# mako443/Text2Pos-CVPR2022

Measured on AMD Instinct MI355X. Metric: cells+queries encoded/sec and top-k retrieval QPS, 256-pt cells, 12k-cell DB, higher is better.
Workload: dtype f16x3 (fp32 operands split hi+lo into fp16, 3 f16 MFMAs, fp32 accumulate; fp32-class error) for the encoders / f64 MFMA for the ranking

## Files before the change

### include/t2p.h

```cpp
#ifndef T2P_H
#define T2P_H
#include <stddef.h>
#include <stdint.h>

#ifdef __cplusplus
extern "C" {
#endif

#define T2P_ABI_VERSION 29
#define T2P_DEFAULT_CHUNK_OBJECTS 65000
#define T2P_MAX_CHUNK_OBJECTS 65535
#define T2P_TUNING_MASK 0x1
#define T2P_E_ARG (-1)
#define T2P_E_WORKSPACE (-2)
#define T2P_E_UNSUPPORTED (-3)

typedef void* t2p_stream_t;

int t2p_abi_version(void);
const char* t2p_last_error(void);

typedef struct t2p_cell_weights {
    const float* sa_w1[3];
    const float* sa_b1[3];
    const float* sa_w2[3];
    const float* sa_b2[3];
    const float* ga_w1;
    const float* ga_b1;
    const float* ga_w2;
    const float* ga_b2;
    const float* lin1_w;
    const float* lin1_b;
    const float* lin2_w;
    const float* lin2_b;
    const float* pn_w;
    const float* pn_b;
    const float* col_w1;
    const float* col_b1;
    const float* col_w2;
    const float* col_b2;
    const float* pos_w1;
    const float* pos_b1;
    const float* pos_w2;
    const float* pos_b2;
    const float* merge_w;
    const float* merge_b;
    const float* g_wp;
    const float* g_bp;
    const float* g_wq;
    const float* g_w2;
    const float* g_b2;
    const float* lin_w1;
    const float* lin_b1;
    const float* lin_w2;
    const float* lin_b2;
    const void* sa_w2_x3[3];
    const void* ga_w2_x3;
    const float* sa_b2_x3[3];
    float sa_w2_scale[3];
    const void* lin1_x3;
    const void* lin2_x3;
    const void* merge_x3;
    const void* pn_x3;
    const void* g_wp_x3;
    const void* g_wq_x3;
// ... 189 lines not shown
```

### text2pos-cvpr2022_amd/csrc/api.hip

```cpp
#include <stdarg.h>
#include <stdlib.h>
#include <string.h>

#include <mutex>
#include <set>
#include <utility>

#include "../../include/t2p.h"
#include "t2p_common.h"

namespace t2p {

static thread_local char g_err[512] = "";

void set_error(const char* fmt, ...) {
    va_list ap;
    va_start(ap, fmt);
    vsnprintf(g_err, sizeof(g_err), fmt, ap);
    va_end(ap);
}

int num_cus() {
    static int cached = 0;
    if (cached == 0) {
// ... 294 lines not shown
            p.W_x3 = cfg.precision == 1 ? W.sa_w1_x3[l] : nullptr;
            p.ldw = H;
            p.bias = W.sa_b1[l];
            p.out = ws.A[l];
            p.ldo = H;
            p.relu = 0;
            p.M = n * g.nd[l];
            p.amax_out = gslot(l == 1 ? G_A2 : G_A3);
            T2P_TRY(launch_ws(WS_DENSE_STORE, Geo::LD[l - 1] - (cfg.precision == 1 ? 16 : 0), H, p, st));
        }
        SaParams p{};
        p.A = ws.A[l];
        p.Bc = ws.B[l];
        p.wp = lds_btab[l] ? W.sa_w1[l] + (size_t)cf * Geo::H[l] : nullptr;
        p.W = W.sa_w2[l];
        p.W_x3 = cfg.precision == 1 ? W.sa_w2_x3[l] : nullptr;
        p.bias = cfg.precision == 1 ? W.sa_b2_x3[l] : W.sa_b2[l];
        p.out_scale = cfg.precision == 1 ? 1.0f / W.sa_w2_scale[l] : 1.0f;
        p.out = ws.F[l];
        p.ldo = Geo::LD[l];
        p.rows = ws.gt.rows[l];
        p.n_rows = ws.gt.n_rows[l];
        p.first = ws.first;
        p.fps_idx = ws.gt.fps_idx[l];
        p.pos_src = pos_src;
        p.ld_pos = ld_pos;
        p.pos_col0 = pos_col0;
        if (l == 0 && sa1_points) {
            p.feat_src = rgb;
            p.w1 = W.sa_w1[0];
            p.b1 = W.sa_b1[0];
        }
        p.n_dense = g.nd[l];
        p.n_cent = g.nc[l];
        p.n_obj = n;
        p.prefix_ws = ws.prefix[l];
        p.bounds_ws = ws.bounds[l];
        p.balanced = 1;
        p.amax_out = gslot(G_F1 + l);
        if (l == 2) p.out_rows = g.gp;
        T2P_TRY(launch_ws_sa(H, C, p, st));
    }
    {
        WsParams p{};
        p.A = ws.F[2];
        p.lda = Geo::LD[2];
        p.W = W.ga_w1;
        p.W_x3 = cfg.precision == 1 ? W.ga_w1_x3 : nullptr;
        p.ldw = 512;
        p.bias = W.ga_b1;
        p.out = ws.gh;
        _Float16* gh_hi = (_Float16*)ws.gh;
        _Float16* gh_lo = gh_hi + (size_t)gh_rows(n, g) * 512;
        if (cfg.precision == 1) {
            p.out_hi = gh_hi;
            p.out_lo = gh_lo;
            p.amax_out = gslot(G_GA_H);
        }
        p.ldo = 512;
        p.relu = 1;
        p.M = n * g.gp;
        T2P_TRY(launch_ws(WS_DENSE_STORE, Geo::LD[2] - (cfg.precision == 1 ? 16 : 0), 512, p, st));
        WsParams q{};
        q.A = ws.gh;
        if (cfg.precision == 1) {
            q.A_hi = gh_hi;
            q.A_lo = gh_lo;
        }
        q.lda = 512;
        q.W = W.ga_w2;
        q.W_x3 = cfg.precision == 1 ? W.ga_w2_x3 : nullptr;
        q.ldw = 1024;
        q.bias = W.ga_b2;
        q.out = ws.f0;
        q.ldo = 1024;
        q.relu = 1;
        q.M = n * g.gp;
        q.group_rows = g.gp;
        T2P_TRY(launch_ws(WS_DENSE_GROUPMAX, 512, 1024, q, st));
    }
    if (cfg.precision == 1 && W.lin1_x3 && W.lin2_x3) {
        T2P_TRY(launch_gemm_x3(ws.f0, 1024, W.lin1_x3, W.lin1_scale, W.lin1_b, ws.f1, 512, 0, n, 1024, 512, 1, st, nullptr, 0, gslot(G_PN_F0)));
        T2P_TRY(launch_gemm_x3(ws.f1, 512, W.lin2_x3, W.lin2_scale, W.lin2_b, ws.f2, 256, 0, n, 512, 256, 1, st, nullptr, 0, gslot(G_PN_F1)));
    } else {
        T2P_TRY(launch_gemm(ws.f0, 1024, W.lin1_w, W.lin1_b, ws.f1, 512, 0, n, 1024, 512, 1, st));
        T2P_TRY(launch_gemm(ws.f1, 512, W.lin2_w, W.lin2_b, ws.f2, 256, 0, n, 512, 256, 1, st));
    }
    }
    if (trunk_only) {
        T2P_TRY(copy_trace(tr->features0, ws.f0, (size_t)n * 1024, st));
        T2P_TRY(copy_trace(tr->features1, ws.f1, (size_t)n * 512, st));
        T2P_TRY(copy_trace(tr->features2, ws.f2, (size_t)n * 256, st));
        T2P_TRY(launch_guard_check(guard, cfg.overflow_flag, gbounds, st));
        return 0;
    }
    const int nfeat = (cfg.use_class ? 1 : 0) + (cfg.use_color ? 1 : 0) + (cfg.use_position ? 1 : 0);
    const int ldcat = nfeat * D;
    int slot = 0;
    if (cfg.use_class && cfg.class_embed) {
        T2P_TRY(launch_gather_rownorm(W.class_embedding, cfg.class_idx + o_lo, n, D, ws.cat, ldcat, slot * D, st));
        slot++;
    } else if (cfg.use_class) {
        const float* fin = cfg.pointnet_features == 0 ? ws.f0 : (cfg.pointnet_features == 1 ? ws.f1 : ws.f2);
        const int kin = cfg.pointnet_features == 0 ? 1024 : (cfg.pointnet_features == 1 ? 512 : 256);
        if (cfg.precision == 1 && W.pn_x3)
            T2P_TRY(launch_gemm_x3(fin, kin, W.pn_x3, W.pn_scale, W.pn_b, ws.P, D, 0, n, kin, D, 1, st, nullptr, 0,
                                          gslot(G_PN_F0 + cfg.pointnet_features)));
        else
            T2P_TRY(launch_gemm(fin, kin, W.pn_w, W.pn_b, ws.P, D, 0, n, kin, D, 1, st));
        T2P_TRY(launch_rownorm(ws.P, D, n, D, ws.cat, ldcat, slot * D, st));
        slot++;
    }
    if (cfg.use_color && cfg.color_embed) {
        T2P_TRY(launch_gather_rownorm(W.color_embedding, cfg.color_idx + o_lo, n, D, ws.cat, ldcat, slot * D, st));
        slot++;
    } else if (cfg.use_color) {
        T2P_TRY(launch_mlp3_norm(mean_rgb, n, W.col_w1, W.col_b1, W.col_w2, W.col_b2, D, ws.cat, ldcat, slot * D, st));
        slot++;
    }
    if (cfg.use_position) {
// ... 643 lines not shown
```

### text2pos-cvpr2022_amd/csrc/ga2.hip

```cpp
#include "t2p_common.h"

namespace t2p {
namespace {

typedef _Float16 half8 __attribute__((ext_vector_type(8)));

constexpr int K = 512, NW = 128, NT = 512;
constexpr int KH = K / 2;
constexpr int S16_FULL = K / 16;
constexpr int LDHH = K + 8;
constexpr int PLANE = 32 * LDHH;
constexpr int TILE_HALVES = 2 * PLANE;
constexpr int XCH_FLOATS = 4 * 16 * 64;
constexpr size_t kLds = (size_t)2 * TILE_HALVES * 2 + (size_t)XCH_FLOATS * 4;
constexpr int CHUNKS = (2 * 32 * (K / 8)) / NT;

template <int GP>
__global__ __launch_bounds__(NT, 2) void k_ga2(WsParams p, int n_slices) {
    extern __shared__ __attribute__((aligned(16))) float lds[];
    _Float16* tile = (_Float16*)lds;
    float* xch = (float*)(tile + 2 * TILE_HALVES);

    const int tid = threadIdx.x, lane = tid & 63, wave = tid >> 6;
    const int wn = wave & 3, kh = wave >> 2;

    const int lin = blockIdx.x, nblk = gridDim.x;
    int slice, stream, n_streams;
    if ((nblk % (8 * n_slices)) == 0) {
        const int xcd = lin & 7, j = lin >> 3, per_xcd = nblk >> 3;
        slice = j % n_slices;
        stream = xcd * (per_xcd / n_slices) + j / n_slices;
        n_streams = nblk / n_slices;
    } else {
        slice = lin % n_slices;
        stream = lin / n_slices;
        n_streams = nblk / n_slices;
    }
    const int ncol0 = slice * NW + wn * 32;

    constexpr int S32 = KH / 32;
    const int q16 = lane >> 4, i16 = lane & 15;
    half8 w_hi[2][S32], w_lo[2][S32];
    {
        const uint4* wp = (const uint4*)p.W_x3;
        const int plane_u4 = (p.ldw / 32) * S16_FULL * 64;
#pragma unroll
        for (int cb = 0; cb < 2; cb++)
#pragma unroll
            for (int s = 0; s < S32; s++) {
                const int idx = (((ncol0 / 32) * S16_FULL + (8 * q16 + s)) * 2 + kh) * 32 + 16 * cb + i16;
                w_hi[cb][s] = __builtin_bit_cast(half8, wp[idx]);
                w_lo[cb][s] = __builtin_bit_cast(half8, wp[plane_u4 + idx]);
            }
    }
    float bias2[2];
#pragma unroll
    for (int cb = 0; cb < 2; cb++) bias2[cb] = p.bias ? p.bias[ncol0 + 16 * cb + i16] : 0.f;

    typedef __attribute__((address_space(3))) void lds_void;
    typedef const __attribute__((address_space(1))) void gl_void;
    auto dma_piece = [&](int64_t g, int buf, int it) {
        const int q = it * (NT / 64) + wave;
        const int pl = q >> 5, row = q & 31;
        const _Float16* base = (const _Float16*)(pl ? p.A_lo : p.A_hi);
        const _Float16* src = base + (g * 32 + row) * (int64_t)p.lda + lane * 8;
        _Float16* dst = tile + buf * TILE_HALVES + pl * PLANE + row * LDHH;
        __builtin_amdgcn_global_load_lds((gl_void*)src, (lds_void*)dst, 16, 0, 0);
    };
    auto dma_tile = [&](int64_t g, int buf) {
#pragma unroll
        for (int it = 0; it < CHUNKS; it++) dma_piece(g, buf, it);
    };
    int64_t g = stream;
    if (g < p.n_groups) dma_tile(g, 0);
    __syncthreads();
    for (int i = 0; g < p.n_groups; g += n_streams, i++) {
        const int64_t gn = g + n_streams;
        const bool more = gn < p.n_groups;

        typedef float f32x4v __attribute__((ext_vector_type(4)));
        const f32x4v kZero4 = {0.f, 0.f, 0.f, 0.f};
        f32x4v acc[4], accx[4];
        const _Float16* hrow = tile + (i & 1) * TILE_HALVES + i16 * LDHH + kh * KH + q16 * 64;
        half8 a_hi[2], a_lo[2];
#pragma unroll
        for (int rb = 0; rb < 2; rb++) {
            a_hi[rb] = *(const half8*)(hrow + rb * 16 * LDHH);
            a_lo[rb] = *(const half8*)(hrow + PLANE + rb * 16 * LDHH);
        }
#pragma unroll
        for (int sl = 0; sl < 4 * S32; sl++) {
            const int s = sl >> 2, b = sl & 3, rb = b >> 1, cb = b & 1;
            __builtin_amdgcn_sched_barrier(0);
            if (s + 1 < S32 && b == 2) {
                a_hi[0] = *(const half8*)(hrow + (s + 1) * 8);
                a_lo[0] = *(const half8*)(hrow + PLANE + (s + 1) * 8);
            }
            if (s > 0 && b == 0) {
                a_hi[1] = *(const half8*)(hrow + 16 * LDHH + s * 8);
                a_lo[1] = *(const half8*)(hrow + PLANE + 16 * LDHH + s * 8);
            }
            acc[b] = __builtin_amdgcn_mfma_f32_16x16x32_f16(a_hi[rb], w_hi[cb][s], s == 0 ? kZero4 : acc[b], 0, 0, 0);
            accx[b] = __builtin_amdgcn_mfma_f32_16x16x32_f16(a_hi[rb], w_lo[cb][s], s == 0 ? kZero4 : accx[b], 0, 0, 0);
            accx[b] = __builtin_amdgcn_mfma_f32_16x16x32_f16(a_lo[rb], w_hi[cb][s], accx[b], 0, 0, 0);
            __builtin_amdgcn_sched_barrier(0);
            if (more && (sl & 1) == 0 && (sl >> 1) < CHUNKS) dma_piece(gn, (i + 1) & 1, sl >> 1);
        }
        __builtin_amdgcn_sched_barrier(0);
#pragma unroll
        for (int b = 0; b < 4; b++)
#pragma unroll
            for (int v = 0; v < 4; v++) acc[b][v] = fmaf(accx[b][v], 1.f / 2048.f, acc[b][v]);
        float* x = xch + wn * (16 * 64) + lane;
        const bool sender = ((i & 1) != 0) == (kh == 0);
        if (sender) {
#pragma unroll
            for (int b = 0; b < 4; b++)
#pragma unroll
                for (int v = 0; v < 4; v++) x[(4 * b + v) * 64] = acc[b][v];
        }
        __syncthreads();
        if (!sender && GP == 32) {
#pragma unroll
            for (int cb = 0; cb < 2; cb++) {
                float m = 0.f;
#pragma unroll
                for (int rb = 0; rb < 2; rb++)
#pragma unroll
                    for (int v = 0; v < 4; v++) m = fmaxf(m, (acc[2 * rb + cb][v] + x[(4 * (2 * rb + cb) + v) * 64]) + bias2[cb]);
                m = fmaxf(m, __shfl_xor(m, 16, 64));
                m = fmaxf(m, __shfl_xor(m, 32, 64));
                if (q16 == 0) p.out[g * (int64_t)p.ldo + ncol0 + 16 * cb + i16] = m;
            }
        } else if (!sender) {
            constexpr int VG = GP < 4 ? GP : 4;
            const int64_t n_obj = p.M / GP;
#pragma unroll
            for (int cb = 0; cb < 2; cb++)
#pragma unroll
                for (int rb = 0; rb < 2; rb++)
#pragma unroll
                    for (int v0 = 0; v0 < 4; v0 += VG) {
                        float m = 0.f;
#pragma unroll
                        for (int v = v0; v < v0 + VG; v++)
                            m = fmaxf(m, (acc[2 * rb + cb][v] + x[(4 * (2 * rb + cb) + v) * 64]) + bias2[cb]);
                        if constexpr (GP >= 8) m = fmaxf(m, __shfl_xor(m, 16, 64));
                        if constexpr (GP >= 16) m = fmaxf(m, __shfl_xor(m, 32, 64));
                        const int row = 16 * rb + 4 * q16 + v0;
                        const int64_t obj = g * (32 / GP) + row / GP;
                        if (row % GP == 0 && obj < n_obj) p.out[obj * (int64_t)p.ldo + ncol0 + 16 * cb + i16] = m;
                    }
        }
    }
}

template <int GP>
int launch_ga2_gp(const WsParams& p_in, hipStream_t st) {
    T2P_TRY(reserve_lds((const void*)k_ga2<GP>, kLds, "ga2"));
    WsParams p = p_in;
    p.n_groups = (p.M + 31) / 32;
    if (p.n_groups <= 0) return 0;
    const int n_slices = 1024 / NW;
    int64_t streams = matrix_wgs() / n_slices;
    if (streams < 1) streams = 1;
    if (streams > p.n_groups) streams = p.n_groups;
    if (streams >= 8) streams -= streams % 8;
    ProfScope ps_("ws_groupmax_k512_n1024", st);
    T2P_REPEAT(ps_) hipLaunchKernelGGL(k_ga2<GP>, dim3((unsigned)(streams * n_slices)), dim3(NT), kLds, st, p, n_slices);
    T2P_CHECK_LAUNCH("ga2");
    return 0;
}

}

int launch_ga2(const WsParams& p, hipStream_t st) {
    switch (p.group_rows > 0 ? p.group_rows : 32) {
        case 32: return launch_ga2_gp<32>(p, st);
        case 16: return launch_ga2_gp<16>(p, st);
        case 8: return launch_ga2_gp<8>(p, st);
        case 4: return launch_ga2_gp<4>(p, st);
        case 2: return launch_ga2_gp<2>(p, st);
        case 1: return launch_ga2_gp<1>(p, st);
    }
    set_error("ga2: group_rows=%d (1, 2, 4, 8, 16 or 32)", p.group_rows);
    return T2P_E_UNSUPPORTED;
}

}
```

### text2pos-cvpr2022_amd/csrc/t2p_common.h

```cpp
#pragma once
#include <hip/hip_runtime.h>
#include <stdint.h>
#include <stdio.h>

namespace t2p {

void set_error(const char* fmt, ...);

#define T2P_E_ARG (-1)
#define T2P_E_WORKSPACE (-2)
#define T2P_E_UNSUPPORTED (-3)

#define T2P_CHECK_ARG(cond, ...)                  \
    do {                                          \
        if (!(cond)) {                            \
            ::t2p::set_error(__VA_ARGS__);        \
            return T2P_E_ARG;                     \
        }                                         \
    } while (0)

#define T2P_CHECK_LAUNCH(name)                                                   \
    do {                                                                         \
        hipError_t e__ = hipGetLastError();                                      \
        if (e__ != hipSuccess) {                                                 \
// ... 123 lines not shown
    float* A1;
    const float* w1;
    const float* b1;
    const float* rgb;
    int H1;
    uint32_t* guard;
};
int launch_sample_group(const float* xyz, int64_t n_obj, int n_pts, const float radius[3], GroupTables gt,
                        hipStream_t st);
int launch_dedup_rows(const float* xyz, const float* rgb, int64_t n_obj, int n_pts, uint16_t* rows, uint16_t* n_rows,
                      int n_cent, hipStream_t st);

int launch_rownorm(const float* in, int ld_in, int64_t n_rows, int dim, float* out, int ld_out, int col0,
                   hipStream_t st);
int launch_gather_rownorm(const float* table, const int32_t* idx, int64_t n_rows, int dim, float* out, int ld_out,
                          int col0, hipStream_t st);
int launch_segmax(const float* in, int dim, const int32_t* seg_ptr, int n_seg, float* out, int mean,
                  hipStream_t st);
int launch_knn(const float* x, int dim, const int32_t* seg_ptr, int n_seg, int max_seg_rows, int k,
               int32_t* out_idx, hipStream_t st);
int launch_mlp3_norm(const float* in3, int64_t n_rows, const float* w1, const float* b1, const float* w2,
                     const float* b2, int D, float* out, int ld_out, int col0, hipStream_t st);
int launch_pack_objects(const float* raw_xyz, const float* raw_rgb, const int32_t* obj_ptr, const int32_t* sample_idx,
                        const float* rot, int64_t n_obj, int n_pts, float* xyz, float* rgb, float* center, float* mean_rgb,
                        hipStream_t st);
int launch_pack_scene(const float* raw_xyz, const float* raw_rgb, const int32_t* obj_ptr, const int32_t* obj_id, const uint64_t* key,
                      const float* scene_center, const float* scene_color, int64_t n_out, int n_pts, float* xyz, float* rgb,
                      float* center, float* mean_rgb, int32_t* idx_out, hipStream_t st);
int launch_pairwise_ranking(const float* scores, int batch, float margin, float* row_loss, float* d_scores, float* row_cnt,
                            hipStream_t st);
int launch_hardest_ranking(const float* scores, int batch, float margin, float* best, int32_t* where, float* d_scores,
                           hipStream_t st);
int launch_cell_index(const int32_t* cell_ptr, int n_cells, int32_t o_lo, int32_t* seg_ptr_local, int32_t* first,
                      hipStream_t st, uint32_t* guard_to_clear = nullptr);

int launch_gemm(const float* A, int lda, const float* W, const float* bias, float* C, int ldc, int c0, int64_t M,
                int K, int N, int relu, hipStream_t st, const float* resid = nullptr, int ldr = 0);
int launch_gemm_skinny(const float* A, int lda, const float* W, float* C, int ldc, int64_t M, int K, int N, hipStream_t st);
int launch_gemm_x3(const float* A, int lda, const void* Wx, float scale, const float* bias, float* C, int ldc, int c0,
                   int64_t M, int K, int N, int relu, hipStream_t st, const float* resid = nullptr, int ldr = 0,
                   uint32_t* amax_in = nullptr );

size_t gemm_tn_workspace_bytes(int64_t M, int K1, int N);
int launch_edge_counts(const uint16_t* rows, const uint16_t* n_rows, const int32_t* first_obj, int64_t n_obj, int n_dense, int n_cent,
                       int self_loops, int32_t* counts, hipStream_t st);
int launch_edge_expand(const uint16_t* rows, const uint16_t* n_rows, const int32_t* first_obj, const int32_t* cent_ptr, int64_t n_obj,
                       int n_dense, int n_cent, int self_loops, int32_t* src, int32_t* dst, hipStream_t st);
size_t linear_wgrad_workspace_bytes(int64_t M, int K1, int N);
int launch_linear_wgrad_f32(const float* dY, int lda, const float* X, int ldb, float* dW, int ldc, float* colsum, int64_t M, int K1, int N,
                            void* ws, size_t ws_bytes, hipStream_t st);
int launch_gemm_tn(const float* A, int lda, const float* B, int ldb, float* C, int ldc, int64_t M, int K1, int N, void* ws,
                   size_t ws_bytes, hipStream_t st);

enum WsMode { WS_DENSE_STORE = 0, WS_DENSE_GROUPMAX = 1, WS_EDGE_KNN = 3 };
struct WsParams {
    const float* A;
    int lda;
    int k_live;
    const float* Bc;
    const float* W;
    int ldw;
    const void* W_x3;
    const void* A_hi;
    const void* A_lo;
    void* out_hi;
    void* out_lo;
    const float* bias;
    float* out;
    int ldo;
    int relu;
    int64_t n_groups;
    int64_t M;
    uint32_t* amax_out;
    const int32_t* knn_idx;
    int knn_k;
    int64_t n_dst;
    int mean;
    int knn_group;
    int group_rows;
};
int launch_ws(int mode, int K, int N, const WsParams& p, hipStream_t st);

struct SaParams {
    const float* A;
    const float* Bc;
    const float* wp;
    const float* W;
    const void* W_x3;
    const float* bias;
    float out_scale;
    float* out;
    int ldo;
    const uint16_t* rows;
    const uint16_t* n_rows;
    const int32_t* first;
    const uint8_t* fps_idx;
    const float* pos_src;
    int ld_pos, pos_col0;
    const float* feat_src;
    const float* w1;
    const float* b1;
    int n_dense, n_cent;
    int64_t n_obj;
    int32_t* prefix_ws;
    int32_t* bounds_ws;
    int balanced;
    uint32_t* amax_out;
    int out_rows;
};
int launch_ws_sa(int H, int C, const SaParams& p, hipStream_t st);
int launch_sa_x3(int H, int C, const SaParams& p, hipStream_t st);
int sa_x3_launch_shape(int H, int C, int64_t n_obj, int* tile_rows, int* n_wg);
bool sa_rows_selected(int H, int C, const SaParams& p);
int launch_sa_rows(int H, int C, const SaParams& p, hipStream_t st);
int sa_rows_launch_shape(int64_t n_obj, int* tile_rows, int* n_wg);
bool sa_points_selected(int H, int C, const SaParams& p);
int launch_sa_points(int H, int C, const SaParams& p, hipStream_t st);
int sa_points_launch_shape(int64_t n_obj, int* tile_rows, int* n_wg);
bool sa3_selected(int H, int C, const SaParams& p);
// ... 48 lines not shown
```

### text2pos-cvpr2022_amd/csrc/ws_gemm.hip

```cpp
#ifndef T2P_GABL
#define T2P_GABL 0
#endif
#ifndef T2P_GA2_V1
#define T2P_GA2_V1 0
#endif
#include <type_traits>

#include "t2p_common.h"

namespace t2p {
namespace {

typedef _Float16 half8 __attribute__((ext_vector_type(8)));
typedef __fp16 fp16x2 __attribute__((ext_vector_type(2)));

constexpr int kMaxRows = 32 * 33;
constexpr int kAccFloats = 8192;

template <int K, int NW, int WN, int RT, int MODE, int X3, int W8 = 0>
struct WsCfg {
    static constexpr int NWAVES = (WN > 4 || W8) ? 8 : 4;
    static constexpr int NTH = 64 * NWAVES;
    static constexpr int WM = NWAVES / WN;
    static constexpr int NTW = NW / (32 * WN);
// ... 51 lines not shown
    half8 w_hi[X3 ? C::NTW : 1][X3 ? C::S16 : 1], w_lo[X3 ? C::NTW : 1][X3 ? C::S16 : 1];
    if constexpr (X3) {
        const uint4* wp = (const uint4*)p.W_x3;
        const int plane_u4 = (p.ldw / 32) * C::S16 * 64;
#pragma unroll
        for (int nt = 0; nt < C::NTW; nt++)
#pragma unroll
            for (int s = 0; s < C::S16; s++) {
                const int idx = (((ncol0 / 32 + nt) * C::S16 + s) * 2 + h) * 32 + l31;
                const uint4 a = wp[idx], b = wp[plane_u4 + idx];
                w_hi[nt][s] = __builtin_bit_cast(half8, a);
                w_lo[nt][s] = __builtin_bit_cast(half8, b);
            }
    } else {
#pragma unroll
        for (int nt = 0; nt < C::NTW; nt++)
#pragma unroll
            for (int s = 0; s < C::KS; s++)
                w[nt][s] = p.W[(int64_t)(h * C::KS + s) * p.ldw + ncol0 + nt * 32 + l31];
    }
    float bias[C::NTW];
#pragma unroll
    for (int nt = 0; nt < C::NTW; nt++) bias[nt] = p.bias ? p.bias[ncol0 + nt * 32 + l31] : 0.f;

    const int k_live = p.k_live > 0 ? p.k_live : K;
    f32x4 sa[C::ITERS];
    f32x4 sb[C::EDGE ? C::ITERS : 1];

    const int knn_group = (C::EDGE && p.knn_group > 0) ? p.knn_group : 32;
    auto stage_load = [&](int64_t g, int r0, int n_rows) {
#pragma unroll
        for (int it = 0; it < C::ITERS; it++) {
            const int q = it * C::NTH + tid;
            const int lr = q / C::F4_PER_ROW, c4 = q % C::F4_PER_ROW;
            const int r = r0 + lr;
            sa[it] = f32x4{0.f, 0.f, 0.f, 0.f};
            if constexpr (C::EDGE) sb[it] = f32x4{0.f, 0.f, 0.f, 0.f};
            if (((C::TOTAL_F4 % C::NTH) == 0 || q < C::TOTAL_F4) && (r < n_rows || SPLIT_IO == 1)) {
                if constexpr (C::EDGE) {
                    const int src = rows_src[r];
                    const int dl = rows_dst[r];
                    if (dl != 0xFF) {
                        sa[it] = *(const f32x4*)(p.A + (int64_t)src * p.lda + c4 * 4);
                        sb[it] = *(const f32x4*)(p.Bc + (g * knn_group + dl) * K + c4 * 4);
                    }
                } else if constexpr (SPLIT_IO == 1) {
                    constexpr int CH_PER_PLANE = C::TR * (K / 8);
                    const int pl = q / CH_PER_PLANE, idx = q % CH_PER_PLANE;
                    const int prow = idx / (K / 8), c8 = idx % (K / 8);
                    const _Float16* base = (const _Float16*)(pl ? p.A_lo : p.A_hi);
                    sa[it] = f32x4{0.f, 0.f, 0.f, 0.f};
                    if (prow < n_rows) sa[it] = *(const f32x4*)(base + (g * C::TR + prow) * (int64_t)p.lda + c8 * 8);
                } else {
                    if (SPLIT_IO == 2 || c4 * 4 < k_live)
                        sa[it] = *(const f32x4*)(p.A + (g * C::TR + r) * (int64_t)p.lda + c4 * 4);
                }
            }
        }
    };
    float gmax_edge = 0.f;
    auto stage_write = [&](int buf) {
#pragma unroll
        for (int it = 0; it < C::ITERS; it++) {
            const int q = it * C::NTH + tid;
            if ((C::TOTAL_F4 % C::NTH) != 0 && q >= C::TOTAL_F4) break;
            const int lr = q / C::F4_PER_ROW, c4 = q % C::F4_PER_ROW;
            f32x4 v = sa[it];
            if constexpr (C::EDGE) {
                const f32x4 t = sa[it] + sb[it];
#pragma unroll
                for (int e = 0; e < 4; e++) v[e] = fmaxf(t[e], 0.f);
            }
            if constexpr (X3 && SPLIT_IO == 1) {
                constexpr int CH_PER_PLANE = C::TR * (K / 8);
                const int pl = q / CH_PER_PLANE, idx = q % CH_PER_PLANE;
                const int prow = idx / (K / 8), c8 = idx % (K / 8);
                *(f32x4*)(hidh + buf * 2 * C::PLANE + pl * C::PLANE + prow * C::LDHH + c8 * 8) = sa[it];
            } else if constexpr (X3) {
                _Float16* dsth = hidh + buf * 2 * C::PLANE;
                if constexpr (C::EDGE)
                    gmax_edge = fmaxf(fmaxf(gmax_edge, fmaxf(v[0], v[1])), fmaxf(v[2], v[3]));
                const fp16x2 h01 = cvt_pk_f16(v[0], v[1]), h23 = cvt_pk_f16(v[2], v[3]);
                const fp16x2 l01 = cvt_pk_f16((v[0] - (float)h01[0]) * 2048.f, (v[1] - (float)h01[1]) * 2048.f);
                const fp16x2 l23 = cvt_pk_f16((v[2] - (float)h23[0]) * 2048.f, (v[3] - (float)h23[1]) * 2048.f);
                uint2 ph, pl;
                ph.x = __builtin_bit_cast(uint32_t, h01); ph.y = __builtin_bit_cast(uint32_t, h23);
                pl.x = __builtin_bit_cast(uint32_t, l01); pl.y = __builtin_bit_cast(uint32_t, l23);
                *(uint2*)(dsth + lr * C::LDHH + c4 * 4) = ph;
                *(uint2*)(dsth + C::PLANE + lr * C::LDHH + c4 * 4) = pl;
            } else {
                *(f32x4*)(hid + buf * C::TILE_FLOATS + lr * C::LDH + c4 * 4) = v;
            }
        }
    };
    auto mfma_block = [&](int buf, f32x16 (&acc)[RT][C::NTW]) {
#pragma unroll
        for (int rt = 0; rt < RT; rt++)
#pragma unroll
            for (int nt = 0; nt < C::NTW; nt++)
#pragma unroll
                for (int e = 0; e < 16; e++) acc[rt][nt][e] = bias[nt];
        if constexpr (X3) {
            f32x16 accx[RT][C::NTW];
#pragma unroll
            for (int rt = 0; rt < RT; rt++)
#pragma unroll
                for (int nt = 0; nt < C::NTW; nt++)
// ... 50 lines not shown
#pragma unroll
                for (int rt = 0; rt < RT; rt++) a[rt] = *(const f32x4*)(hrow + rt * 32 * C::LDH + s4 * 4);
#pragma unroll
                for (int j = 0; j < 4; j++)
#pragma unroll
                    for (int rt = 0; rt < RT; rt++)
#pragma unroll
                        for (int nt = 0; nt < C::NTW; nt++)
                            acc[rt][nt] = __builtin_amdgcn_mfma_f32_32x32x2f32(a[rt][j], w[nt][s4 * 4 + j], acc[rt][nt],
                                                                                0, 0, 0);
            }
        }
    };

    if constexpr (!C::EDGE) {
        int64_t g = stream;
        auto rows_of = [&](int64_t gg) -> int {
            const int64_t left = p.M - gg * C::TR;
            return (int)(left < C::TR ? left : C::TR);
        };
        if (g < p.n_groups) {
            stage_load(g, 0, rows_of(g));
            stage_write(0);
        }
        __syncthreads();
        float gmax_all = 0.f;
        (void)gmax_all;
        for (int i = 0; g < p.n_groups; g += n_streams, i++) {
            const int64_t gn = g + n_streams;
            const int n_rows = rows_of(g);
            if (gn < p.n_groups) stage_load(gn, 0, rows_of(gn));
            f32x16 acc[RT][C::NTW];
            mfma_block(i & 1, acc);
            float gmax_out = 0.f;
            (void)gmax_out;
            auto epilogue = [&](auto full_tag) {
            constexpr bool FULL = decltype(full_tag)::value;
#pragma unroll
            for (int rt = 0; rt < RT; rt++) {
                const int trow0 = (wm * RT + rt) * 32;
#pragma unroll
                for (int nt = 0; nt < C::NTW; nt++) {
                    const int lcol = wn * C::NTW * 32 + nt * 32 + l31;
                    if constexpr (MODE == WS_DENSE_STORE) {
                        const int64_t o0 = (g * C::TR + trow0 + 4 * h) * (int64_t)p.ldo + slice * NW + lcol;
#pragma unroll
                        for (int e = 0; e < 16; e++) {
                            const int rr = (e & 3) + 8 * (e >> 2);
                            const int r = trow0 + 4 * h + rr;
                            float v = acc[rt][nt][e];
                            if (p.relu) v = fmaxf(v, 0.f);
                            if constexpr (X3) gmax_out = fmaxf(gmax_out, fabsf(v));
                            if constexpr (SPLIT_IO == 2) {
                                const fp16x2 hv = cvt_pk_f16(v, 0.f);
                                const fp16x2 lv = cvt_pk_f16((v - (float)hv[0]) * 2048.f, 0.f);
#if T2P_GABL & 1
                                if (FULL || r < n_rows) {
                                    ((__fp16*)p.out_hi + (o0 & 0xFFFFF))[rr * p.ldo] = hv[0];
                                    ((__fp16*)p.out_lo + (o0 & 0xFFFFF))[rr * p.ldo] = lv[0];
                                }
#else
                                if (FULL || r < n_rows) {
                                    ((__fp16*)p.out_hi + o0)[rr * p.ldo] = hv[0];
                                    ((__fp16*)p.out_lo + o0)[rr * p.ldo] = lv[0];
                                }
#endif
                            } else {
                                if (FULL || r < n_rows) (p.out + o0)[rr * p.ldo] = v;
                            }
                        }
                    } else if constexpr (GP == 32) {
                        float m = 0.f;
#pragma unroll
                        for (int e = 0; e < 16; e++) m = fmaxf(m, acc[rt][nt][e]);
                        m = fmaxf(m, __shfl_xor(m, 32, 64));
                        if (h == 0 && (FULL || trow0 < n_rows))
                            p.out[(g * (C::TR / 32) + wm * RT + rt) * (int64_t)p.ldo + slice * NW + lcol] = m;
                    } else {
                        constexpr int NG = 32 / GP;
                        float mg[NG];
#pragma unroll
                        for (int k = 0; k < NG; k++) mg[k] = 0.f;
#pragma unroll
                        for (int e = 0; e < 16; e++) {
                            const int k = (8 * (e >> 2) + (GP >= 8 ? 0 : (e & 3))) / GP;
                            mg[k] = fmaxf(mg[k], acc[rt][nt][e]);
                        }
                        const int64_t obj0 = (g * C::TR + trow0) / GP, n_obj = p.M / GP;
#pragma unroll
                        for (int k = 0; k < NG; k++) {
                            if constexpr (GP >= 8) {
                                const float m = fmaxf(mg[k], __shfl_xor(mg[k], 32, 64));
                                if (h == 0 && obj0 + k < n_obj) p.out[(obj0 + k) * (int64_t)p.ldo + slice * NW + lcol] = m;
                            } else if ((k * GP) % 8 < 4) {
                                const int64_t obj = obj0 + k + (4 / GP) * h;
                                if (obj < n_obj) p.out[obj * (int64_t)p.ldo + slice * NW + lcol] = mg[k];
                            }
                        }
                    }
                }
            }
            };
            if (n_rows == C::TR) epilogue(std::true_type{});
            else epilogue(std::false_type{});
            if constexpr (X3 && MODE == WS_DENSE_STORE) gmax_all = fmaxf(gmax_all, gmax_out);
            if (gn < p.n_groups) stage_write((i + 1) & 1);
            __syncthreads();
        }
        if constexpr (X3 && MODE == WS_DENSE_STORE) guard_publish_exact(p.amax_out, gmax_all);
    } else {
        for (int64_t g = stream; g < p.n_groups; g += n_streams) {
            const int64_t d0 = g * knn_group;
            const int nd = (int)((p.n_dst - d0) < knn_group ? (p.n_dst - d0) : knn_group);
            int my = 0;
            if (tid < nd)
                for (int e = 0; e < p.knn_k; e++) my += p.knn_idx[(d0 + tid) * p.knn_k + e] >= 0 ? 1 : 0;
            if (tid <= 32) scan[tid] = 0;
            __syncthreads();
            if (tid < 32) scan[tid + 1] = my;
// ... 79 lines not shown
                        for (int e = 0; e < 16; e++)
                            if (is_end[e]) atomicMax(&acc_lds[dd[e] * NW + lcol], __float_as_int(v[e]));
                    }
                }
                if (more) stage_write((bt + 1) & 1);
                __syncthreads();
            }
            for (int i = tid; i < nd * NW; i += C::NTH) {
                const int c = i / NW, col = i % NW;
                p.out[(d0 + c) * (int64_t)p.ldo + slice * NW + col] = __int_as_float(acc_lds[i]);
            }
            __syncthreads();
        }
        if constexpr (X3) guard_publish_exact(p.amax_out, gmax_edge);
    }
}

template <int K, int NW, int WN, int RT, int MODE, int X3, int SPLIT_IO, int W8 = 0, int GP = 32>
int launch_cfg(const WsParams& p_in, int n_slices, hipStream_t st) {
    using C = WsCfg<K, NW, WN, RT, MODE, X3, W8>;
    auto kern = k_ws<K, NW, WN, RT, MODE, X3, SPLIT_IO, W8, GP>;
    T2P_TRY(reserve_lds((const void*)kern, C::lds_bytes(), "ws_gemm"));
    WsParams p = p_in;
    if (MODE != WS_EDGE_KNN) p.n_groups = (p.M + C::TR - 1) / C::TR;
    if (p.n_groups <= 0) return 0;
    const int cus = num_cus();
    int64_t streams = cus / n_slices;
    if (streams < 1) streams = 1;
    if (streams > p.n_groups) streams = p.n_groups;
    if (streams >= 8) streams -= streams % 8;
    const unsigned grid = (unsigned)(streams * n_slices);
    static const char* kMode[] = {"dense", "groupmax", "edge_sa", "edge_knn"};
    static char name[64];
    if (name[0] == 0) snprintf(name, sizeof(name), "ws_%s_k%d_n%d", kMode[MODE], K, NW * n_slices);
    ProfScope ps_(name, st);
    T2P_REPEAT(ps_) hipLaunchKernelGGL(kern, dim3(grid), dim3(C::NTH), C::lds_bytes(), st, p, n_slices);
    T2P_CHECK_LAUNCH("ws_gemm");
    return 0;
}

}

int launch_ga2(const WsParams& p, hipStream_t st);

int launch_ws(int mode, int K, int N, const WsParams& p, hipStream_t st) {
    T2P_CHECK_ARG((((uintptr_t)p.A | (uintptr_t)p.A_hi | (uintptr_t)p.A_lo) & 15) == 0 && (p.lda % 4) == 0,
                  "ws_gemm: A must be 16-byte aligned, lda %% 4 == 0");
    const int x3 = p.W_x3 != nullptr ? 1 : 0;
    if (x3) T2P_CHECK_ARG(((uintptr_t)p.W_x3 & 15) == 0, "ws_gemm: packed f16x3 weights must be 16-byte aligned");
    const int gp = p.group_rows > 0 ? p.group_rows : 32;
    if (mode == WS_DENSE_GROUPMAX)
        T2P_CHECK_ARG(gp <= 32 && (gp & (gp - 1)) == 0 && p.M % gp == 0, "ws_gemm: groupmax needs group_rows in {1, 2, 4, 8, 16, 32} "
                      "and M %% group_rows == 0 (group_rows=%d M=%lld)", p.group_rows, (long long)p.M);
    const int split_io = p.A_hi != nullptr ? 1 : (p.out_hi != nullptr ? 2 : 0);
    T2P_CHECK_ARG(split_io == 0 || x3 == 1, "ws_gemm: split fp16 activations need the f16x3 path");
    T2P_CHECK_ARG(p.k_live == 0 || (split_io == 0 && mode == WS_DENSE_STORE && p.k_live % 4 == 0),
                  "ws_gemm: k_live is honoured by the fp32-in / fp32-out dense mode only (multiple of 4)");
    if (split_io == 1) T2P_CHECK_ARG(p.A_lo != nullptr && p.lda % 8 == 0, "ws_gemm: split input needs both planes, lda %% 8 == 0");
    if (split_io == 2) T2P_CHECK_ARG(p.out_lo != nullptr, "ws_gemm: split output needs both planes");
#define WS_CASE(MODE_, K_, N_, NW_, WN_, RT_, X3_, SIO_)                                      \
    if (mode == MODE_ && K == K_ && N == N_ && x3 == X3_ && split_io == SIO_)                  \
        return launch_cfg<K_, NW_, WN_, RT_, MODE_, X3_, SIO_>(p, N_ / NW_, st);
    WS_CASE(WS_EDGE_KNN, 256, 256, 256, 8, 1, 0, 0)
    WS_CASE(WS_EDGE_KNN, 256, 256, 256, 8, 1, 1, 0)
    WS_CASE(WS_EDGE_KNN, 128, 128, 128, 4, 1, 0, 0)
    WS_CASE(WS_EDGE_KNN, 128, 128, 128, 4, 1, 1, 0)
    WS_CASE(WS_EDGE_KNN, 384, 384, 128, 4, 1, 0, 0)
    WS_CASE(WS_EDGE_KNN, 384, 384, 128, 4, 1, 1, 0)
    WS_CASE(WS_DENSE_STORE, 96, 128, 128, 4, 2, 0, 0)
    WS_CASE(WS_DENSE_STORE, 160, 256, 256, 4, 1, 0, 0)
    WS_CASE(WS_DENSE_STORE, 288, 512, 128, 4, 1, 0, 0)
    if (mode == WS_DENSE_STORE && K == 80 && N == 128 && x3 == 1 && split_io == 0)
        return launch_cfg<80, 128, 4, 1, WS_DENSE_STORE, 1, 0, 1>(p, 1, st);
    WS_CASE(WS_DENSE_STORE, 144, 256, 256, 8, 1, 1, 0)
    WS_CASE(WS_DENSE_STORE, 272, 512, 256, 8, 1, 1, 2)
    if (mode == WS_DENSE_GROUPMAX && K == 512 && N == 1024 && x3 == 0 && split_io == 0) {
        switch (gp) {
            case 32: return launch_cfg<512, 128, 4, 1, WS_DENSE_GROUPMAX, 0, 0>(p, 8, st);
            case 16: return launch_cfg<512, 128, 4, 1, WS_DENSE_GROUPMAX, 0, 0, 0, 16>(p, 8, st);
            case 8: return launch_cfg<512, 128, 4, 1, WS_DENSE_GROUPMAX, 0, 0, 0, 8>(p, 8, st);
            case 4: return launch_cfg<512, 128, 4, 1, WS_DENSE_GROUPMAX, 0, 0, 0, 4>(p, 8, st);
            case 2: return launch_cfg<512, 128, 4, 1, WS_DENSE_GROUPMAX, 0, 0, 0, 2>(p, 8, st);
            case 1: return launch_cfg<512, 128, 4, 1, WS_DENSE_GROUPMAX, 0, 0, 0, 1>(p, 8, st);
        }
    }
#if !T2P_GA2_V1
    if (mode == WS_DENSE_GROUPMAX && K == 512 && N == 1024 && x3 == 1 && split_io == 1) return launch_ga2(p, st);
#endif
    T2P_CHECK_ARG(mode != WS_DENSE_GROUPMAX || gp == 32, "ws_gemm: group_rows=%d is built for the fp32 and the ga2.hip paths", gp);
    WS_CASE(WS_DENSE_GROUPMAX, 512, 1024, 128, 4, 1, 1, 1)
#undef WS_CASE
    set_error("ws_gemm: no instantiation for mode=%d K=%d N=%d x3=%d split_io=%d", mode, K, N, x3, split_io);
    return T2P_E_UNSUPPORTED;
}

}
```

Measured before the change: 148,900.

## Store GA hidden fp16 planes in swizzled line-blocked tiles for ga2 loads

Changes the layout of the split hi/lo fp16 hidden activations between the two GA layers. Instead of row-major planes, they are stored as 32-row by 512-column tiles made of 32x32 blocks with an XOR swizzle. The producer GEMM writes them with buffer stores, and the ga2 group-max kernel DMA-loads each tile as contiguous memory into LDS, where it reads the operand pieces without bank conflicts and without row padding. The old row-major path stays available behind tuning bit 4. The risk is that the producer's scattered 2-byte stores become less coalesced.

```diff
diff --git a/include/t2p.h b/include/t2p.h
--- a/include/t2p.h
+++ b/include/t2p.h
@@ -10,7 +10,7 @@
 #define T2P_ABI_VERSION 29
 #define T2P_DEFAULT_CHUNK_OBJECTS 65000
 #define T2P_MAX_CHUNK_OBJECTS 65535
-#define T2P_TUNING_MASK 0x1
+#define T2P_TUNING_MASK 0x5
 #define T2P_E_ARG (-1)
 #define T2P_E_WORKSPACE (-2)
 #define T2P_E_UNSUPPORTED (-3)
diff --git a/text2pos-cvpr2022_amd/csrc/api.hip b/text2pos-cvpr2022_amd/csrc/api.hip
--- a/text2pos-cvpr2022_amd/csrc/api.hip
+++ b/text2pos-cvpr2022_amd/csrc/api.hip
@@ -370,9 +370,11 @@
         p.out = ws.gh;
         _Float16* gh_hi = (_Float16*)ws.gh;
         _Float16* gh_lo = gh_hi + (size_t)gh_rows(n, g) * 512;
+        const int gh_rowmajor = (cfg.tuning & 4) ? 1 : 0;
         if (cfg.precision == 1) {
             p.out_hi = gh_hi;
             p.out_lo = gh_lo;
+            p.plane_rowmajor = gh_rowmajor;
             p.amax_out = gslot(G_GA_H);
         }
         p.ldo = 512;
@@ -384,6 +386,7 @@
         if (cfg.precision == 1) {
             q.A_hi = gh_hi;
             q.A_lo = gh_lo;
+            q.plane_rowmajor = gh_rowmajor;
         }
         q.lda = 512;
         q.W = W.ga_w2;
diff --git a/text2pos-cvpr2022_amd/csrc/ga2.hip b/text2pos-cvpr2022_amd/csrc/ga2.hip
--- a/text2pos-cvpr2022_amd/csrc/ga2.hip
+++ b/text2pos-cvpr2022_amd/csrc/ga2.hip
@@ -9,14 +9,19 @@
 constexpr int KH = K / 2;
 constexpr int S16_FULL = K / 16;
 constexpr int LDHH = K + 8;
-constexpr int PLANE = 32 * LDHH;
-constexpr int TILE_HALVES = 2 * PLANE;
 constexpr int XCH_FLOATS = 4 * 16 * 64;
-constexpr size_t kLds = (size_t)2 * TILE_HALVES * 2 + (size_t)XCH_FLOATS * 4;
 constexpr int CHUNKS = (2 * 32 * (K / 8)) / NT;
-
-template <int GP>
+static_assert(K == kGaPlaneCols, "the line-blocked planes are K columns wide");
+template <bool LINES>
+struct Tile {
+    static constexpr int PLANE = LINES ? kGaTileHalves : 32 * LDHH;
+    static constexpr int TILE_HALVES = 2 * PLANE;
+    static constexpr size_t kLds = (size_t)2 * TILE_HALVES * 2 + (size_t)XCH_FLOATS * 4;
+};
+
+template <int GP, bool LINES>
 __global__ __launch_bounds__(NT, 2) void k_ga2(WsParams p, int n_slices) {
+    constexpr int PLANE = Tile<LINES>::PLANE, TILE_HALVES = Tile<LINES>::TILE_HALVES;
     extern __shared__ __attribute__((aligned(16))) float lds[];
     _Float16* tile = (_Float16*)lds;
     float* xch = (float*)(tile + 2 * TILE_HALVES);
@@ -63,8 +68,9 @@
         const int q = it * (NT / 64) + wave;
         const int pl = q >> 5, row = q & 31;
         const _Float16* base = (const _Float16*)(pl ? p.A_lo : p.A_hi);
-        const _Float16* src = base + (g * 32 + row) * (int64_t)p.lda + lane * 8;
-        _Float16* dst = tile + buf * TILE_HALVES + pl * PLANE + row * LDHH;
+        const _Float16* src = LINES ? base + g * kGaTileHalves + row * (kGaBlockHalves / 2) + lane * 8
+                                    : base + (g * 32 + row) * (int64_t)p.lda + lane * 8;
+        _Float16* dst = tile + buf * TILE_HALVES + pl * PLANE + row * (LINES ? kGaBlockHalves / 2 : LDHH);
         __builtin_amdgcn_global_load_lds((gl_void*)src, (lds_void*)dst, 16, 0, 0);
     };
     auto dma_tile = [&](int64_t g, int buf) {
@@ -82,23 +88,32 @@
         const f32x4v kZero4 = {0.f, 0.f, 0.f, 0.f};
         f32x4v acc[4], accx[4];
         const _Float16* hrow = tile + (i & 1) * TILE_HALVES + i16 * LDHH + kh * KH + q16 * 64;
+        const _Float16* hpc[4];
+#pragma unroll
+        for (int pc = 0; pc < 4; pc++)
+            hpc[pc] = tile + (i & 1) * TILE_HALVES + ((kh * KH + q16 * 64) / 32) * kGaBlockHalves + ga_block_off(i16, 8 * pc);
+        static_assert(ga_block_off(16, 0) == kGaBlockHalves / 2, "rows 16-31 of a block follow rows 0-15");
+        auto opnd = [&](int s, int rb, int pl) -> half8 {
+            if constexpr (LINES) return *(const half8*)(hpc[s & 3] + pl * PLANE + rb * (kGaBlockHalves / 2) + (s >> 2) * kGaBlockHalves);
+            else return *(const half8*)(hrow + pl * PLANE + rb * 16 * LDHH + s * 8);
+        };
         half8 a_hi[2], a_lo[2];
 #pragma unroll
         for (int rb = 0; rb < 2; rb++) {
-            a_hi[rb] = *(const half8*)(hrow + rb * 16 * LDHH);
-            a_lo[rb] = *(const half8*)(hrow + PLANE + rb * 16 * LDHH);
+            a_hi[rb] = opnd(0, rb, 0);
+            a_lo[rb] = opnd(0, rb, 1);
         }
 #pragma unroll
         for (int sl = 0; sl < 4 * S32; sl++) {
             const int s = sl >> 2, b = sl & 3, rb = b >> 1, cb = b & 1;
             __builtin_amdgcn_sched_barrier(0);
             if (s + 1 < S32 && b == 2) {
-                a_hi[0] = *(const half8*)(hrow + (s + 1) * 8);
-                a_lo[0] = *(const half8*)(hrow + PLANE + (s + 1) * 8);
+                a_hi[0] = opnd(s + 1, 0, 0);
+                a_lo[0] = opnd(s + 1, 0, 1);
             }
             if (s > 0 && b == 0) {
-                a_hi[1] = *(const half8*)(hrow + 16 * LDHH + s * 8);
-                a_lo[1] = *(const half8*)(hrow + PLANE + 16 * LDHH + s * 8);
+                a_hi[1] = opnd(s, 1, 0);
+                a_lo[1] = opnd(s, 1, 1);
             }
             acc[b] = __builtin_amdgcn_mfma_f32_16x16x32_f16(a_hi[rb], w_hi[cb][s], s == 0 ? kZero4 : acc[b], 0, 0, 0);
             accx[b] = __builtin_amdgcn_mfma_f32_16x16x32_f16(a_hi[rb], w_lo[cb][s], s == 0 ? kZero4 : accx[b], 0, 0, 0);
@@ -155,9 +170,10 @@
     }
 }
 
-template <int GP>
+template <int GP, bool LINES>
 int launch_ga2_gp(const WsParams& p_in, hipStream_t st) {
-    T2P_TRY(reserve_lds((const void*)k_ga2<GP>, kLds, "ga2"));
+    constexpr size_t kLds = Tile<LINES>::kLds;
+    T2P_TRY(reserve_lds((const void*)k_ga2<GP, LINES>, kLds, "ga2"));
     WsParams p = p_in;
     p.n_groups = (p.M + 31) / 32;
     if (p.n_groups <= 0) return 0;
@@ -167,21 +183,27 @@
     if (streams > p.n_groups) streams = p.n_groups;
     if (streams >= 8) streams -= streams % 8;
     ProfScope ps_("ws_groupmax_k512_n1024", st);
-    T2P_REPEAT(ps_) hipLaunchKernelGGL(k_ga2<GP>, dim3((unsigned)(streams * n_slices)), dim3(NT), kLds, st, p, n_slices);
+    T2P_REPEAT(ps_) hipLaunchKernelGGL((k_ga2<GP, LINES>), dim3((unsigned)(streams * n_slices)), dim3(NT), kLds, st, p, n_slices);
     T2P_CHECK_LAUNCH("ga2");
     return 0;
 }
 
+template <int GP>
+int launch_ga2_layout(const WsParams& p, hipStream_t st) {
+    return p.plane_rowmajor ? launch_ga2_gp<GP, false>(p, st) : launch_ga2_gp<GP, true>(p, st);
+}
+
 }
 
 int launch_ga2(const WsParams& p, hipStream_t st) {
+    T2P_CHECK_ARG(p.plane_rowmajor || p.lda == kGaPlaneCols, "ga2: line-blocked planes are %d columns wide (lda=%d)", kGaPlaneCols, p.lda);
     switch (p.group_rows > 0 ? p.group_rows : 32) {
-        case 32: return launch_ga2_gp<32>(p, st);
-        case 16: return launch_ga2_gp<16>(p, st);
-        case 8: return launch_ga2_gp<8>(p, st);
-        case 4: return launch_ga2_gp<4>(p, st);
-        case 2: return launch_ga2_gp<2>(p, st);
-        case 1: return launch_ga2_gp<1>(p, st);
+        case 32: return launch_ga2_layout<32>(p, st);
+        case 16: return launch_ga2_layout<16>(p, st);
+        case 8: return launch_ga2_layout<8>(p, st);
+        case 4: return launch_ga2_layout<4>(p, st);
+        case 2: return launch_ga2_layout<2>(p, st);
+        case 1: return launch_ga2_layout<1>(p, st);
     }
     set_error("ga2: group_rows=%d (1, 2, 4, 8, 16 or 32)", p.group_rows);
     return T2P_E_UNSUPPORTED;
diff --git a/text2pos-cvpr2022_amd/csrc/t2p_common.h b/text2pos-cvpr2022_amd/csrc/t2p_common.h
--- a/text2pos-cvpr2022_amd/csrc/t2p_common.h
+++ b/text2pos-cvpr2022_amd/csrc/t2p_common.h
@@ -199,6 +199,48 @@
 int launch_gemm_tn(const float* A, int lda, const float* B, int ldb, float* C, int ldc, int64_t M, int K1, int N, void* ws,
                    size_t ws_bytes, hipStream_t st);
 
+constexpr int kGaPlaneCols = 512;
+constexpr int kGaTileHalves = 32 * kGaPlaneCols;
+constexpr int kGaBlockHalves = 32 * 32;
+__host__ __device__ constexpr int ga_line_of_row(int r) { return (r & 3) + 4 * ((r >> 3) & 3); }
+__host__ __device__ constexpr int ga_half_of_row(int r) { return (r >> 2) & 1; }
+__host__ __device__ constexpr int ga_line_swz(int e) { return (e & 7) >> 1; }
+__host__ __device__ constexpr int ga_lane_off(int h, int c, int swz) { return h * 32 + ((((c >> 3) & 3) ^ swz) << 3) + (c & 7); }
+__host__ __device__ constexpr int ga_block_off(int r, int c) {
+    return ga_line_of_row(r) * 64 + ga_lane_off(ga_half_of_row(r), c, ga_line_swz(ga_line_of_row(r)));
+}
+__host__ __device__ constexpr int64_t ga_plane_off(int64_t row, int col) {
+    return (row >> 5) * kGaTileHalves + (col >> 5) * kGaBlockHalves + ga_block_off((int)(row & 31), col & 31);
+}
+namespace ga_plane_check {
+constexpr bool bijective() {
+    bool seen[kGaBlockHalves] = {};
+    for (int r = 0; r < 32; r++)
+        for (int c = 0; c < 32; c++) {
+            const int o = ga_block_off(r, c);
+            if (o < 0 || o >= kGaBlockHalves || seen[o]) return false;
+            if ((o >= kGaBlockHalves / 2) != (r >= 16)) return false;
+            if ((o >> 6) != ga_line_of_row(r)) return false;
+            if ((c & 7) && o != ga_block_off(r, c - 1) + 1) return false;
+            seen[o] = true;
+        }
+    return true;
+}
+constexpr bool conflict_free() {
+    for (int rb = 0; rb < 2; rb++)
+        for (int piece = 0; piece < 4; piece++) {
+            unsigned quads = 0;
+            for (int i = 0; i < 16; i++) quads |= 1u << ((ga_block_off(16 * rb + i, 8 * piece) >> 3) & 15);
+            if (quads != 0xFFFFu) return false;
+        }
+    return true;
+}
+static_assert(bijective(), "ga_block_off must be a bijection of a 32 x 32 block onto its 16 lines");
+static_assert(conflict_free(), "ga_block_off must spread the 16 rows of an operand block over all LDS banks");
+static_assert(ga_plane_off(32, 0) == kGaTileHalves && ga_plane_off(0, 32) == kGaBlockHalves && ga_plane_off(31, 511) < 2 * kGaTileHalves,
+              "tiles of 32 KB, blocks of 2 KB");
+}
+
 enum WsMode { WS_DENSE_STORE = 0, WS_DENSE_GROUPMAX = 1, WS_EDGE_KNN = 3 };
 struct WsParams {
     const float* A;
@@ -212,6 +254,7 @@
     const void* A_lo;
     void* out_hi;
     void* out_lo;
+    int plane_rowmajor;
     const float* bias;
     float* out;
     int ldo;
diff --git a/text2pos-cvpr2022_amd/csrc/ws_gemm.hip b/text2pos-cvpr2022_amd/csrc/ws_gemm.hip
--- a/text2pos-cvpr2022_amd/csrc/ws_gemm.hip
+++ b/text2pos-cvpr2022_amd/csrc/ws_gemm.hip
@@ -127,7 +127,7 @@
                     sa[it] = f32x4{0.f, 0.f, 0.f, 0.f};
                     if (prow < n_rows) sa[it] = *(const f32x4*)(base + (g * C::TR + prow) * (int64_t)p.lda + c8 * 8);
                 } else {
-                    if (SPLIT_IO == 2 || c4 * 4 < k_live)
+                    if (SPLIT_IO >= 2 || c4 * 4 < k_live)
                         sa[it] = *(const f32x4*)(p.A + (g * C::TR + r) * (int64_t)p.lda + c4 * 4);
                 }
             }
@@ -284,19 +284,29 @@
                             if (p.relu) v = fmaxf(v, 0.f);
                             if constexpr (X3) gmax_out = fmaxf(gmax_out, fabsf(v));
                             if constexpr (SPLIT_IO == 2) {
+                                static_assert(C::TR == 32 && NW * 2 == kGaPlaneCols, "the line-blocked planes hold 32-row tiles of 512 columns");
                                 const fp16x2 hv = cvt_pk_f16(v, 0.f);
                                 const fp16x2 lv = cvt_pk_f16((v - (float)hv[0]) * 2048.f, 0.f);
+                                const int wn_u = __builtin_amdgcn_readfirstlane(wn);
+                                int64_t blk = g * kGaTileHalves + ((slice * NW + wn_u * C::NTW * 32) / 32 + nt) * kGaBlockHalves;
 #if T2P_GABL & 1
+                                blk &= 0xFFC00;
+#endif
+                                const uint32_t off = (uint32_t)(ga_lane_off(h, l31, 0) ^ (ga_line_swz(e) << 3)) * 2u;
+                                static_assert(ga_lane_off(1, 21, 3) == (ga_lane_off(1, 21, 0) ^ (3 << 3)), "the piece XOR is an XOR of the offset");
+                                const auto rh = __builtin_amdgcn_make_buffer_rsrc((__fp16*)p.out_hi + blk, 0, kGaBlockHalves * 2, 0x00020000);
+                                const auto rl = __builtin_amdgcn_make_buffer_rsrc((__fp16*)p.out_lo + blk, 0, kGaBlockHalves * 2, 0x00020000);
                                 if (FULL || r < n_rows) {
-                                    ((__fp16*)p.out_hi + (o0 & 0xFFFFF))[rr * p.ldo] = hv[0];
-                                    ((__fp16*)p.out_lo + (o0 & 0xFFFFF))[rr * p.ldo] = lv[0];
+                                    __builtin_amdgcn_raw_buffer_store_b16((short)__builtin_bit_cast(uint32_t, hv), rh, off, e * 128, 0);
+                                    __builtin_amdgcn_raw_buffer_store_b16((short)__builtin_bit_cast(uint32_t, lv), rl, off, e * 128, 0);
                                 }
-#else
+                            } else if constexpr (SPLIT_IO == 3) {
+                                const fp16x2 hv = cvt_pk_f16(v, 0.f);
+                                const fp16x2 lv = cvt_pk_f16((v - (float)hv[0]) * 2048.f, 0.f);
                                 if (FULL || r < n_rows) {
                                     ((__fp16*)p.out_hi + o0)[rr * p.ldo] = hv[0];
                                     ((__fp16*)p.out_lo + o0)[rr * p.ldo] = lv[0];
                                 }
-#endif
                             } else {
                                 if (FULL || r < n_rows) (p.out + o0)[rr * p.ldo] = v;
                             }
@@ -482,12 +492,14 @@
     if (mode == WS_DENSE_GROUPMAX)
         T2P_CHECK_ARG(gp <= 32 && (gp & (gp - 1)) == 0 && p.M % gp == 0, "ws_gemm: groupmax needs group_rows in {1, 2, 4, 8, 16, 32} "
                       "and M %% group_rows == 0 (group_rows=%d M=%lld)", p.group_rows, (long long)p.M);
-    const int split_io = p.A_hi != nullptr ? 1 : (p.out_hi != nullptr ? 2 : 0);
+    const int split_io = p.A_hi != nullptr ? 1 : (p.out_hi != nullptr ? (p.plane_rowmajor ? 3 : 2) : 0);
     T2P_CHECK_ARG(split_io == 0 || x3 == 1, "ws_gemm: split fp16 activations need the f16x3 path");
     T2P_CHECK_ARG(p.k_live == 0 || (split_io == 0 && mode == WS_DENSE_STORE && p.k_live % 4 == 0),
                   "ws_gemm: k_live is honoured by the fp32-in / fp32-out dense mode only (multiple of 4)");
     if (split_io == 1) T2P_CHECK_ARG(p.A_lo != nullptr && p.lda % 8 == 0, "ws_gemm: split input needs both planes, lda %% 8 == 0");
-    if (split_io == 2) T2P_CHECK_ARG(p.out_lo != nullptr, "ws_gemm: split output needs both planes");
+    if (split_io >= 2) T2P_CHECK_ARG(p.out_lo != nullptr, "ws_gemm: split output needs both planes");
+    if (split_io == 2) T2P_CHECK_ARG(p.ldo == kGaPlaneCols && N == kGaPlaneCols, "ws_gemm: line-blocked planes are %d columns wide (ldo=%d N=%d)",
+                                     kGaPlaneCols, p.ldo, N);
 #define WS_CASE(MODE_, K_, N_, NW_, WN_, RT_, X3_, SIO_)                                      \
     if (mode == MODE_ && K == K_ && N == N_ && x3 == X3_ && split_io == SIO_)                  \
         return launch_cfg<K_, NW_, WN_, RT_, MODE_, X3_, SIO_>(p, N_ / NW_, st);
@@ -504,6 +516,7 @@
         return launch_cfg<80, 128, 4, 1, WS_DENSE_STORE, 1, 0, 1>(p, 1, st);
     WS_CASE(WS_DENSE_STORE, 144, 256, 256, 8, 1, 1, 0)
     WS_CASE(WS_DENSE_STORE, 272, 512, 256, 8, 1, 1, 2)
+    WS_CASE(WS_DENSE_STORE, 272, 512, 256, 8, 1, 1, 3)
     if (mode == WS_DENSE_GROUPMAX && K == 512 && N == 1024 && x3 == 0 && split_io == 0) {
         switch (gp) {
             case 32: return launch_cfg<512, 128, 4, 1, WS_DENSE_GROUPMAX, 0, 0>(p, 8, st);
@@ -518,6 +531,7 @@
     if (mode == WS_DENSE_GROUPMAX && K == 512 && N == 1024 && x3 == 1 && split_io == 1) return launch_ga2(p, st);
 #endif
     T2P_CHECK_ARG(mode != WS_DENSE_GROUPMAX || gp == 32, "ws_gemm: group_rows=%d is built for the fp32 and the ga2.hip paths", gp);
+    T2P_CHECK_ARG(split_io != 1 || p.plane_rowmajor, "ws_gemm: the split-input kernel reads row-major planes only (tuning bit 2)");
     WS_CASE(WS_DENSE_GROUPMAX, 512, 1024, 128, 4, 1, 1, 1)
 #undef WS_CASE
     set_error("ws_gemm: no instantiation for mode=%d K=%d N=%d x3=%d split_io=%d", mode, K, N, x3, split_io);
```

After: 149,700, median of 6. No clear change (+0.5%).
